# JiYuanFeng/DDP

Hardware: AMD Instinct MI355X
Metric: images/s at K DDIM steps (512x1024, 150-class) per GPU and whole node (higher is better)
Workload: dtype f32 (bf16x3-split MFMA products, fp32 accumulate); 1 GPU; ade_swin_t_k3_8x512x1024 (ADE20K Swin-T DDP decode head, 3-step DDIM, batch 8x512x1024 per GPU; x (8,256,128,256), random-init weights); images_per_call=8, ddim_steps=3, parallelism=dp1 (independent images, weights broadcast once), gemm_engine=bf16x3

## Files before the change

ddp_amd/csrc/ddp_api.hip:

```cpp
#include <stdarg.h>
#include <stdio.h>
#include <string.h>

#include <cmath>
#include <initializer_list>

#include "ddp_internal.h"

namespace ddp {

static thread_local char g_err[512] = "";

void set_error(const char* fmt, ...) {
  va_list ap;
  va_start(ap, fmt);
  vsnprintf(g_err, sizeof(g_err), fmt, ap);
  va_end(ap);
}

int check_launch(const char* what) {
  hipError_t e = hipGetLastError();
  if (e != hipSuccess) {
    set_error("%s: %s", what, hipGetErrorString(e));
    return DDP_E_LAUNCH;
// ... 515 lines not shown
  return DDP_OK;
}

int fold_affine_dev(const ddp_weights* w, int L, int S, const float* film, float* aff, hipStream_t st) {
  for (int l = 0; l < L; ++l) {
    const ddp_layer_weights& lw = w->layers[l];
    for (int s = 0; s < S; ++s) {
      float* dst = aff + (size_t(s) * L + l) * 512;
      if (lw.time_w && film) {
        DDP_TRY(launch_fold_affine(lw.norm1_w, lw.norm1_b, film + (size_t(s) * L + l) * 512, dst, 1, st));
      } else {
        DDP_TRY(launch_pack_rows(lw.norm1_w, 1, lw.norm1_b, 1, dst, 256, st));
      }
    }
  }
  return DDP_OK;
}

int prepare_geometry(const Layout& o, hipStream_t st) {
  for (int l = 0; l < o.L; ++l) DDP_TRY(launch_pos_tables(o.wcat[l], o.bcat[l], o.py[l], o.px[l], o.hh, o.wh, st));
  if (o.b3 && hipMemsetAsync(o.vpad, 0, o.vpad_floats * sizeof(float), st) != hipSuccess) {
    set_error("hipMemsetAsync(vpad) failed");
    return DDP_E_LAUNCH;
  }
  if (o.rvpad && hipMemsetAsync(o.rvpad, 0, o.vpad_floats * sizeof(float), st) != hipSuccess) {
    set_error("hipMemsetAsync(rvpad) failed");
    return DDP_E_LAUNCH;
  }
  return DDP_OK;
}

struct BiasSeg {
  int at;
  const float* src;
  int n;
};
int bias_table(float* dst, std::initializer_list<BiasSeg> segs, const char* what, hipStream_t st) {
  bool ok = hipMemsetAsync(dst, 0, size_t(b3_layer_bias_floats()) * sizeof(float), st) == hipSuccess;
  for (const BiasSeg& s : segs)
    ok = ok && (!s.src || hipMemcpyAsync(dst + s.at, s.src, size_t(s.n) * sizeof(float), hipMemcpyDeviceToDevice, st) == hipSuccess);
  if (!ok) {
    set_error("%s: bias table copy failed", what);
    return DDP_E_LAUNCH;
  }
  return DDP_OK;
}

int build_proj_images(const Layout& o, int l, unsigned char* stream, int base, hipStream_t st) {
  DDP_TRY(launch_build_stages(o.wp_v[l].p, o.wp_v[l].comp_stride, 256, 256, 1, 4, 2, base, 0, 1, 2, stream, st));
  DDP_TRY(launch_build_stages(o.wp_cat[l].p, o.wp_cat[l].comp_stride, 256, 96, 1, 1, 2, base + 8, 0, 1, 2, stream, st));
  return launch_build_stages(o.wp_cat[l].p, o.wp_cat[l].comp_stride, 256, 96, 2, 1, 1, base + 10, 64, 0, 0, stream, st);
}

int prepare_model(const ddp_cfg* c, const ddp_weights* w, const Layout& o, hipStream_t st) {
  DDP_TRY(launch_pack_cols(w->transform_w, o.Cx + o.Cm, 0, 256, o.Cx, o.wx, st));
  DDP_TRY(launch_pack_cols(w->transform_w, o.Cx + o.Cm, o.Cx, 256, o.Cm, o.wm, st));
  if (c->task == DDP_TASK_SEG) DDP_TRY(launch_build_lut(w->embedding, o.lut, o.Kc + 1, c->bit_scale, st));
  if (c->task == DDP_TASK_DEPTH) DDP_TRY(launch_pack_conv3x3(w->head_w, o.wtap, st));
  if (o.seg3) {
    if (hipMemsetAsync(o.bins_wpack, 0, size_t(256) * 2304 * sizeof(float), st) != hipSuccess ||
        hipMemsetAsync(o.bins_bias, 0, 256 * sizeof(float), st) != hipSuccess ||
        hipMemcpyAsync(o.bins_bias, w->head_b, size_t(o.Kc) * sizeof(float), hipMemcpyDeviceToDevice, st) != hipSuccess) {
      set_error("bev 3x3 conv_seg: weight copy failed");
      return DDP_E_LAUNCH;
    }
    DDP_TRY(launch_pack_conv3x3_scaled(w->head_w, nullptr, o.bins_wpack, o.Kc, 256, st));
    if (o.b3) {
      DDP_TRY(launch_split_weights(o.bins_wpack, 2304, 256, 2304, o.bins_wsplit, st));
      DDP_TRY(launch_build_stages(o.bins_wsplit, size_t(256) * 2304, 2304, 256, 0, 1, 72, 0, 2, 1, 0, o.bins_stream, st));
    }
  }
  if (o.nbins) {
    if (hipMemsetAsync(o.bins_wpack, 0, size_t(256) * 2304 * sizeof(float), st) != hipSuccess ||
        hipMemsetAsync(o.bins_bias, 0, 256 * sizeof(float), st) != hipSuccess ||
        hipMemsetAsync(o.bins_tab, 0, DDP_MAX_DEPTH_BINS * sizeof(float), st) != hipSuccess ||
        hipMemcpyAsync(o.bins_bias, w->head_b, size_t(o.nbins) * sizeof(float), hipMemcpyDeviceToDevice, st) != hipSuccess ||
        hipMemcpyAsync(o.bins_tab, w->depth_bins, size_t(o.nbins) * sizeof(float), hipMemcpyDeviceToDevice, st) != hipSuccess) {
      set_error("depth bins: weight copy failed");
      return DDP_E_LAUNCH;
    }
    DDP_TRY(launch_pack_conv3x3_scaled(w->head_w, nullptr, o.bins_wpack, o.nbins, 256, st));
    if (o.b3) {
      DDP_TRY(launch_split_weights(o.bins_wpack, 2304, 256, 2304, o.bins_wsplit, st));
      DDP_TRY(launch_build_stages(o.bins_wsplit, size_t(256) * 2304, 2304, 256, 0, 1, 72, 0, 2, 1, 0, o.bins_stream, st));
    }
  }
  for (int l = 0; l < o.L; ++l) {
    const ddp_layer_weights& lw = w->layers[l];
    DDP_TRY(launch_pack_rows(lw.sampling_offsets_w, 64, lw.attention_weights_w, 32, o.wcat[l], 256, st));
    DDP_TRY(launch_pack_rows(lw.sampling_offsets_b, 64, lw.attention_weights_b, 32, o.bcat[l], 1, st));
  }
  if (o.b3) {
    auto wr = [](const SplitW& w) { return const_cast<unsigned short*>(w.p); };
    DDP_TRY(launch_split_weights(o.wx, o.Cx, 256, o.Cx, wr(o.wp_x), st));
    if (c->task != DDP_TASK_DEPTH) DDP_TRY(launch_split_weights(o.wm, 256, 256, 256, wr(o.wp_m), st));
    if (c->task == DDP_TASK_DEPTH) DDP_TRY(launch_split_weights(o.wtap, 256, 9, 256, wr(o.wp_head), st));
    else if (!o.seg3) DDP_TRY(launch_split_weights(w->head_w, 256, o.Kc, 256, wr(o.wp_head), st));
    for (int l = 0; l < o.L; ++l) {
      const ddp_layer_weights& lw = w->layers[l];
      DDP_TRY(launch_split_weights(lw.value_proj_w, 256, 256, 256, wr(o.wp_v[l]), st));
      DDP_TRY(launch_split_weights(o.wcat[l], 256, 96, 256, wr(o.wp_cat[l]), st));
      DDP_TRY(launch_split_weights(lw.output_proj_w, 256, 256, 256, wr(o.wp_o[l]), st));
      DDP_TRY(launch_split_weights(lw.ffn0_w, 256, DDP_FFN, 256, wr(o.wp_f0[l]), st));
      DDP_TRY(launch_split_weights(lw.ffn1_w, DDP_FFN, 256, DDP_FFN, wr(o.wp_f1[l]), st));
    }
    if (c->task == DDP_TASK_SEG) {
      const int nch = (o.Kc + 63) / 64;
      DDP_TRY(launch_build_stages(o.wp_head.p, o.wp_head.comp_stride, 256, o.Kc, 1, nch, 2, 0, 0, 1, 2, o.tail_stream, st));
      DDP_TRY(bias_table(o.tail_bias, {{0, w->head_b, o.Kc}}, "seg tail", st));
      DDP_TRY(launch_build_stages(o.wp_head.p, o.wp_head.comp_stride, 256, o.Kc, 1, nch, 2, 0, 0, 1, 2, o.tail4_stream, st));
      DDP_TRY(build_proj_images(o, 0, o.tail4_stream, 2 * nch, st));
      DDP_TRY(bias_table(o.tail4_bias, {{0, w->head_b, o.Kc}, {DDP_FFN, w->layers[0].value_proj_b, 256}}, "fused tail", st));
      DDP_TRY(launch_linear(o.lut, 256, false, o.wm, 256, nullptr, nullptr, 0, 0, 0, o.tlut, 256, o.Kc + 1, 256, 256, 0, st));
    }
    if (c->task != DDP_TASK_DEPTH)
      DDP_TRY(launch_build_stages(o.wp_m.p, o.wp_m.comp_stride, 256, 256, 0, 1, 8, 0, 2, 1, 0, o.pro_stream, st));
    DDP_TRY(build_proj_images(o, 0, o.pro_stream, 8, st));
    DDP_TRY(bias_table(o.pro_bias, {{DDP_FFN, w->layers[0].value_proj_b, 256}}, "prologue", st));
    if (o.head7_stream) {
      DDP_TRY(launch_build_stages(o.wp_m.p, o.wp_m.comp_stride, 256, 256, 0, 1, 8, 0, 2, 1, 0, o.head7_stream, st));
      DDP_TRY(launch_build_stages(o.wp_x.p, o.wp_x.comp_stride, 256, 256, 0, 1, 8, 8, 2, 1, 0, o.head7_stream, st));
      if (hipMemcpyAsync(o.head7_stream + size_t(16) * 48 * 1024, o.pro_stream + size_t(8) * 48 * 1024, size_t(11) * 48 * 1024,
                         hipMemcpyDeviceToDevice, st) != hipSuccess) {
        set_error("first-step head stream copy failed");
        return DDP_E_LAUNCH;
      }
    }
    for (int l = 0; l < o.L; ++l) {
      const ddp_layer_weights& lw = w->layers[l];
      unsigned char* sp = o.wstream[l];
      DDP_TRY(launch_build_stages(o.wp_o[l].p, o.wp_o[l].comp_stride, 256, 256, 0, 1, 8, 0, 2, 1, 0, sp, st));
      DDP_TRY(launch_build_stages(o.wp_f0[l].p, o.wp_f0[l].comp_stride, 256, DDP_FFN, 1, 16, 2, 8, 0, 1, 4, sp, st));
      DDP_TRY(launch_build_stages(o.wp_f1[l].p, o.wp_f1[l].comp_stride, DDP_FFN, 256, 0, 1, 32, 10, 4, 1, 0, sp, st));
      DDP_TRY(bias_table(o.bias_ext[l], {{0, lw.ffn0_b, DDP_FFN}}, "layer", st));
      if (l + 1 < o.L) {
        DDP_TRY(build_proj_images(o, l + 1, sp, 72, st));
        if (hipMemcpyAsync(o.bias_ext[l] + DDP_FFN, w->layers[l + 1].value_proj_b, 256 * sizeof(float), hipMemcpyDeviceToDevice, st) !=
            hipSuccess) {
          set_error("bias table copy failed");
          return DDP_E_LAUNCH;
        }
      }
    }
    if (o.lt_stream && c->task != DDP_TASK_SEG && !o.seg3) {
      const size_t sb = size_t(48) * 1024;
      const int rows = c->task == DDP_TASK_DEPTH ? 9 : o.Kc;
      DDP_TRY(launch_build_stages(o.wp_head.p, o.wp_head.comp_stride, 256, rows, 1, 1, 2, 0, 0, 1, 2, o.tail_stream, st));
      DDP_TRY(bias_table(o.tail_bias, {{0, c->task == DDP_TASK_BEV ? w->head_b : nullptr, o.Kc}}, "head tail", st));
      if (hipMemcpyAsync(o.lt_stream, o.wstream[o.L - 1], 72 * sb, hipMemcpyDeviceToDevice, st) != hipSuccess ||
          hipMemcpyAsync(o.lt_stream + 72 * sb, o.tail_stream, 2 * sb, hipMemcpyDeviceToDevice, st) != hipSuccess) {
        set_error("layer + tail stream copy failed");
        return DDP_E_LAUNCH;
      }
      DDP_TRY(bias_table(o.lt_bias, {{0, w->layers[o.L - 1].ffn0_b, DDP_FFN}}, "layer + tail", st));
    }
    if (o.wvs) {
      DDP_TRY(launch_matvec(w->layers[0].value_proj_w, nullptr, o.wm, o.wvs, 256, 256, 1, 256, 256, 0, 0, st));
      DDP_TRY(launch_matvec(o.wcat[0], nullptr, o.wm, o.wvs + 256, 256, 96, 1, 256, 96, 0, 0, st));
    }
    if (o.lut64) {
      DDP_TRY(launch_build_bev_lut(w->embedding, o.lut64, o.Kc, c->bit_scale, st));
      DDP_TRY(launch_linear(o.lut64, 256, false, o.wm, 256, nullptr, nullptr, 0, 0, 0, o.tlut, 256, 1 << o.Kc, 256, 256, 0, st));
    }
    if (o.lt_stream && c->task == DDP_TASK_SEG) {
      const int nch = (o.Kc + 63) / 64;
      const size_t sb = size_t(48) * 1024;
      if (hipMemcpyAsync(o.lt_stream, o.wstream[o.L - 1], 72 * sb, hipMemcpyDeviceToDevice, st) != hipSuccess ||
          hipMemcpyAsync(o.lt_stream + 72 * sb, o.tail4_stream, size_t(2 * nch + 11) * sb, hipMemcpyDeviceToDevice, st) != hipSuccess) {
        set_error("layer + tail stream copy failed");
        return DDP_E_LAUNCH;
      }
      DDP_TRY(bias_table(o.lt_bias, {{0, w->layers[o.L - 1].ffn0_b, DDP_FFN}, {DDP_FFN, w->layers[0].value_proj_b, 256}}, "layer + tail",
                         st));
    }
  }
  return DDP_OK;
}

int publish_q(const Layout& o, const float* row_major, hipStream_t st) {
  if (o.b3 && !o.fused_layer) return launch_row_to_sb(row_major, 256, o.q_sb, int(o.M), 256, st);
  return launch_row_to_blk(row_major, o.q, int(o.M), st);
}

int conv3x3_head(const Layout& o, int n_out, int* layout, int* ld, hipStream_t st) {
  const int M = int(o.M);
  if (o.b3) {
    if (!o.fused_layer) {
      DDP_TRY(launch_sb_to_row(o.q_sb, o.s, M, 256, st));
      DDP_TRY(launch_row_to_blk(o.s, o.q, M, st));
    }
    SgemmProblem pr{};
    pr.A = o.q;
    pr.out = o.bins_logits;
    pr.stream = o.bins_stream;
    pr.M = M;
    pr.ns = 72;
    pr.conv_h = o.hh;
    pr.conv_w = o.wh;
    pr.bias = o.bins_bias;
    prof_begin(TAG_HEAD, st);
    DDP_TRY(launch_b3_sgemm(&pr, 1, 0, 1, st));
    prof_end(TAG_HEAD, st);
    *layout = 0;
    *ld = 256;
  } else {
    DDP_TRY(launch_blk_to_pad(o.q, o.bins_in, o.R, o.hh, o.wh, o.bins_guard, st));
    const int rows = o.R * (o.hh + 2) * (o.wh + 2);
    for (int t = 0; t < 9; ++t) {
      const int off = (t / 3 - 1) * (o.wh + 2) + (t % 3 - 1);
      DDP_TRY(launch_linear(o.bins_in + size_t(o.bins_guard + off) * 256, 256, false, o.bins_wpack + t * 256, 2304,
                            t == 0 ? o.bins_bias : nullptr, t == 0 ? nullptr : o.bins_logits, o.bins_ld, 0, 0, o.bins_logits,
                            o.bins_ld, rows, n_out, 256, 0, st));
    }
    *layout = 1;
    *ld = o.bins_ld;
  }
  return DDP_OK;
}

int depth_bins_head(const ddp_cfg* c, const Layout& o, float* pred, hipStream_t st) {
  DepthBinsArgs a;
// ... 1780 lines not shown
```

ddp_amd/csrc/ddp_internal.h:

```cpp
#pragma once
#include <hip/hip_runtime.h>
#include <stddef.h>
#include <atomic>
#include "../../include/ddp_mi355x.h"


#ifndef DDP_S_F32
#define DDP_S_F32 1
#endif

namespace ddp {

__device__ __forceinline__ float sigmoidf_(float x) { return 1.0f / (1.0f + expf(-x)); }

void set_error(const char* fmt, ...);
int check_launch(const char* what);

struct LdsAttrOnce {
  std::atomic<unsigned long long> done{0};
  void ensure(const void* fn, int bytes) {
    int dev = 0;
    (void)hipGetDevice(&dev);
    if (dev >= 0 && dev < 64 && ((done.load(std::memory_order_acquire) >> dev) & 1ull)) return;
    if (hipFuncSetAttribute(fn, hipFuncAttributeMaxDynamicSharedMemorySize, bytes) != hipSuccess) {
// ... 1 lines not shown
      set_error("hipFuncSetAttribute(MaxDynamicSharedMemorySize = %d) failed on device %d", bytes, dev);
      return;
    }
    if (dev >= 0 && dev < 64) done.fetch_or(1ull << dev, std::memory_order_release);
  }
};
inline int cu_count() {
  static std::atomic<int> cache[64];
  int dev = 0;
  (void)hipGetDevice(&dev);
  if (dev >= 0 && dev < 64) {
    const int c = cache[dev].load(std::memory_order_relaxed);
    if (c > 0) return c;
  }
  int n = 0;
  if (hipDeviceGetAttribute(&n, hipDeviceAttributeMultiprocessorCount, dev) != hipSuccess || n <= 0) n = 256;
  if (dev >= 0 && dev < 64) cache[dev].store(n, std::memory_order_relaxed);
  return n;
}

enum GemmTag {
  TAG_GENERIC = 0, TAG_XPROJ = 1, TAG_FEAT = 2, TAG_VALUE = 3, TAG_SAMP = 4, TAG_OUTPROJ_LN = 5, TAG_FC1 = 6,
  TAG_FC2_LN = 7, TAG_HEAD = 8, TAG_GATHER = 9, TAG_LAYER_TAIL = 10, TAG_COUNT = 11
};
void prof_begin(int tag, hipStream_t st);
void prof_end(int tag, hipStream_t st);

int launch_linear(const float* A, int lda, bool a_blk, const float* W, int ldw, const float* bias, const float* add,
                  int ld_add, int rn, int n_tok, float* out, int ldo, int M, int N, int K, int gelu, hipStream_t st,
                  int tag = TAG_GENERIC);
int launch_linear_blk(const float* A, int lda, bool a_blk, const float* W, int ldw, const float* bias,
                      const float* add, int ld_add, int rn, int n_tok, float* out_blk, int M, int N, int K, int gelu,
                      hipStream_t st);
int launch_linear_res_ln_blk(const float* A, int lda, bool a_blk, const float* W, int ldw, const float* bias,
                             const float* res_blk, const float* ga_aff, const float* be_aff, float* out_blk, int M,
                             int K, hipStream_t st);
int launch_linear_samp(const float* A_blk, const float* Wcat, const float* py, const float* px, int n_tok, int w,
                       float* out, int M, hipStream_t st);

struct SplitW {
  const unsigned short* p;
  size_t comp_stride;
};
int launch_b3_linear(const unsigned short* A_sb, const SplitW& w, const float* bias, const float* add, int ld_add,
                     int rn, int n_tok, float* out, int ldo, int M, int N, int K, hipStream_t st, int tag);
int launch_b3_linear_sb(const unsigned short* A_sb, const SplitW& w, const float* bias, const float* add, int ld_add,
                        int rn, int n_tok, unsigned short* out_sb, float* out_f32_blk, int M, int N, int K, int gelu,
                        hipStream_t st, int tag);
int launch_b3_linear_res_ln(const unsigned short* A_sb, const SplitW& w, const float* bias, const float* res_blk,
                            const unsigned short* res_sb, const float* ga_aff, const float* be_aff, float* out_f32_blk,
                            unsigned short* out_sb, int M, int K, hipStream_t st, int tag);
int launch_b3_linear_samp(const unsigned short* A_sb, const SplitW& wcat, const float* py, const float* px, int n_tok,
                          int w, float* out, int M, hipStream_t st);
int launch_build_stages(const unsigned short* Wp, size_t comp_stride, int K, int rows_valid, int tall, int n_rowblk, int n_kblk,
                        int base, int a, int b, int c, unsigned char* stream, hipStream_t st);
struct LayerLaunch {
  const unsigned short* S;
  const float* Sf;
  float* Q;
  unsigned short* Q_sb;
  const unsigned char* stream;
  const float* bias_ext;
  const float *bo, *ga0, *be0, *b2, *ga1, *be1;
  int M, has_next;
  float* v_out;
  float* samp_out;
  const float *py, *px;
  int n_tok, w;
  const float* res_f;
  const float* wm;
  const float* dvec;
};
int launch_b3_layer(const LayerLaunch& a, hipStream_t st);
struct TailLaunch {
  float* Q;
  const unsigned char* stream;
  const float* bias_ext;
  const float* lut;
  float* prob;
  unsigned short* mask_sb;
  unsigned char* x0_idx;
  const unsigned char* x0_force;
  int x0_keep;
  const float* cp_bias;
  int cp_rn;
  int M, num_classes, ldl, prob_mode;
  float alpha, sigma, alpha_next, sigma_next;
  int fuse_next;
  float* ubuf;
  const float* tlut;
  const float* res;
  int res_rn;
  int res_frag;
  float* v_out;
  float* samp_out;
  const float *py, *px;
  int n_tok, w;
  int kind;
  float threshold;
};
int launch_b3_tail(const TailLaunch& a, hipStream_t st);
bool b3_layer_tail_supported(int num_classes);
int launch_b3_layer_tail(const LayerLaunch& l, const TailLaunch& t, const unsigned char* stream, const float* bias_ext,
                         const float* seg_bias, hipStream_t st);
struct PrologueLaunch {
  const unsigned short* mask_sb;
  float* Q;
  const unsigned char* stream;
// ... 237 lines not shown
```

ddp_amd/csrc/ddp_kernels.hip:

```cpp
#include <math.h>
#include <type_traits>
#include "ddp_internal.h"

namespace ddp {

using f32x4 = __attribute__((ext_vector_type(4))) float;

namespace {

__device__ __forceinline__ float wave_sum(float v) {
#pragma unroll
  for (int o = 32; o > 0; o >>= 1) v += __shfl_xor(v, o, 64);
  return v;
}

__global__ void __launch_bounds__(256) k_nchw_to_tok(const float* __restrict__ in, float* __restrict__ out, int C,
                                                      int N) {
  __shared__ float tile[64][65];
  const int r = blockIdx.z;
  const int n0 = blockIdx.x * 64, c0 = blockIdx.y * 64;
  const int tx = threadIdx.x & 63, ty = threadIdx.x >> 6;
  const float* src = in + size_t(r) * C * N;
  float* dst = out + size_t(r) * N * C;
  for (int cc = ty; cc < 64; cc += 4) {
// ... 1 lines not shown
    tile[cc][tx] = (c < C && n < N) ? src[size_t(c) * N + n] : 0.f;
  }
  __syncthreads();
  for (int nn = ty; nn < 64; nn += 4) {
    const int n = n0 + nn, c = c0 + tx;
    if (n < N && c < C) dst[size_t(n) * C + c] = tile[tx][nn];
  }
}

__device__ __forceinline__ size_t blk_off256(int m, int ch) {
  return size_t(m >> 5) * 8192 + (ch >> 5) * 1024 + ((ch & 31) >> 3) * 256 + ((ch & 7) >> 2) * 128 + (m & 31) * 4 + (ch & 3);
}

__global__ void __launch_bounds__(256) k_row_to_blk(const float* __restrict__ in, float* __restrict__ out, int rows) {
  const int lane = threadIdx.x & 63;
  const int m = blockIdx.x * 4 + (threadIdx.x >> 6);
  if (m >= rows) return;
  const f32x4 v = *reinterpret_cast<const f32x4*>(in + size_t(m) * 256 + lane * 4);
  *reinterpret_cast<f32x4*>(out + blk_off256(m, lane * 4)) = v;
}

__device__ __forceinline__ void split3(float x, unsigned short& p1, unsigned short& p2, unsigned short& p3) {
  const unsigned xb = __float_as_uint(x);
  const unsigned hb = xb & 0xFFFF0000u;
  const float r = x - __uint_as_float(hb);
  const unsigned mb = __float_as_uint(r) & 0xFFFF0000u;
  const float r2 = r - __uint_as_float(mb);
  p1 = (unsigned short)(hb >> 16);
  p2 = (unsigned short)(mb >> 16);
  p3 = (unsigned short)(__float_as_uint(r2) >> 16);
}

__global__ void k_split_weights(const float* __restrict__ W, int ld, int rows, int K, unsigned short* __restrict__ out) {
  const int idx = blockIdx.x * blockDim.x + threadIdx.x;
  const int groups = K / 8;
  if (idx >= rows * groups) return;
  const int row = idx / groups, gq = idx - row * groups;
  const int b = gq >> 1, h = gq & 1;
  const size_t comp = size_t(rows) * K;
  unsigned short* dst = out + size_t(row) * K + 16 * b + 8 * h;
#pragma unroll
  for (int u = 0; u < 8; ++u) {
    const float x = W[size_t(row) * ld + 16 * b + 8 * (u >> 2) + 4 * h + (u & 3)];
    unsigned short p1, p2, p3;
    split3(x, p1, p2, p3);
    dst[u] = p1;
    dst[comp + u] = p2;
    dst[2 * comp + u] = p3;
  }
}

__global__ void __launch_bounds__(256) k_build_stages(const unsigned short* __restrict__ Wp, size_t comp_stride, int K,
                                                       int rows_valid, int tall, int n_kblk, int base, int a, int b, int c,
                                                       unsigned char* __restrict__ stream) {
  const int st = blockIdx.y;
  const int rowblk = st / n_kblk, kblk = st - rowblk * n_kblk;
  const int idx = blockIdx.x * 256 + threadIdx.x;
  if (idx >= 3072) return;
  const int comp = idx >> 10, rem = idx & 1023;
  int row, chunk, slot, grow, kcol;
  if (tall) {
    row = rem >> 4; chunk = rem & 15; slot = chunk ^ (row & 15);
    grow = tall == 2 ? a + (row & 31) : rowblk * 64 + row;
    kcol = (tall == 2 ? (row >> 5) : kblk) * 128 + 8 * chunk;
  } else {
    row = rem >> 2; chunk = rem & 3; slot = chunk ^ ((row >> 2) & 3);
    grow = rowblk * 256 + row;
    kcol = kblk * 32 + 8 * chunk;
  }
  uint4 v = make_uint4(0u, 0u, 0u, 0u);
  if (grow < rows_valid) v = *reinterpret_cast<const uint4*>(Wp + size_t(comp) * comp_stride + size_t(grow) * K + kcol);
  const int image = tall == 2 ? base : base + rowblk * c + (kblk >> 1) * a + (kblk & 1) * b;
  const int per_row = tall ? 16 : 4;
  *reinterpret_cast<uint4*>(stream + size_t(image) * 49152 + comp * 16384 + (row * per_row + slot) * 16) = v;
}

__global__ void __launch_bounds__(256) k_row_to_sb(const float* __restrict__ in, int ld, unsigned short* __restrict__ out,
                                                    int rows, int C) {
  const int slots = C / 8;
  const long idx = long(blockIdx.x) * blockDim.x + threadIdx.x;
  if (idx >= long(rows) * slots) return;
  const int m = int(idx / slots), sl = int(idx - long(m) * slots);
  const int b = sl >> 1, h = sl & 1;
  const float* src = in + size_t(m) * ld + 16 * b + 4 * h;
  const f32x4 lo4 = *reinterpret_cast<const f32x4*>(src);
  const f32x4 hi4 = *reinterpret_cast<const f32x4*>(src + 8);
  unsigned short p[3][8];
#pragma unroll
  for (int u = 0; u < 4; ++u) {
    split3(lo4[u], p[0][u], p[1][u], p[2][u]);
    split3(hi4[u], p[0][4 + u], p[1][4 + u], p[2][4 + u]);
  }
  char* base = reinterpret_cast<char*>(out) + size_t(m >> 5) * C * 192 + size_t(b) * 3 * 1024 + (h * 32 + (m & 31)) * 16;
#pragma unroll
  for (int c = 0; c < 3; ++c) {
    uint4 v;
    v.x = p[c][0] | (unsigned(p[c][1]) << 16);
    v.y = p[c][2] | (unsigned(p[c][3]) << 16);
    v.z = p[c][4] | (unsigned(p[c][5]) << 16);
    v.w = p[c][6] | (unsigned(p[c][7]) << 16);
    *reinterpret_cast<uint4*>(base + c * 1024) = v;
  }
}

__global__ void __launch_bounds__(256) k_nchw_to_sb(const float* __restrict__ in, unsigned short* __restrict__ out, int C, int N,
                                                     int rows) {
  __shared__ float tile[64][65];
  const int m0 = blockIdx.x * 64, c0 = blockIdx.y * 64;
  const int tx = threadIdx.x & 63, ty = threadIdx.x >> 6;
  {
    const int m = m0 + tx;
    const int r = m / N, n = m - r * N;
    const float* src = in + (size_t(r) * C + c0) * N + n;
    for (int cc = ty; cc < 64; cc += 4) tile[cc][tx] = (m < rows && c0 + cc < C) ? src[size_t(cc) * N] : 0.f;
  }
  __syncthreads();
#pragma unroll
  for (int it = 0; it < 2; ++it) {
    const int item = it * 256 + threadIdx.x;
    const int l2 = item & 63, bl = (item >> 6) & 3, gi = item >> 8;
    const int j = l2 & 31, hh = l2 >> 5;
    if (c0 + 16 * bl >= C) continue;
    unsigned short p[3][8];
#pragma unroll
    for (int u = 0; u < 8; ++u) split3(tile[16 * bl + 8 * (u >> 2) + 4 * hh + (u & 3)][gi * 32 + j], p[0][u], p[1][u], p[2][u]);
// ... 1755 lines not shown
  const int Nh = a.hh * a.wh;
  const int m = blockIdx.x * blockDim.x + threadIdx.x;
  if (m >= a.R * Nh) return;
  const float* p;
  if (a.layout == 0) {
    p = a.logits + size_t(m >> 5) * 8192 + (m & 31) * 4;
  } else {
    const int img = m / Nh, n = m - img * Nh;
    const int i = n / a.wh, j = n - i * a.wh;
    p = a.logits + (size_t(img) * (a.hh + 2) * (a.wh + 2) + size_t(i + 1) * (a.wh + 2) + (j + 1)) * a.ld;
  }
  const int K = a.num_classes, nq = (K + 3) >> 2;
  f32x4 v[8];
#pragma unroll
  for (int u = 0; u < 8; ++u) {
    const int q = u < nq ? u : nq - 1;
    const size_t off = a.layout == 0 ? size_t((q >> 1) & 3) * 256 + (q & 1) * 128 : size_t(q) * 4;
    v[u] = *reinterpret_cast<const f32x4*>(p + off);
  }
  float* pr = a.prob + size_t(m) * 32;
  float* lo = a.logits_out ? a.logits_out + size_t(m) * 32 : nullptr;
  unsigned code = 0;
#pragma unroll
  for (int u = 0; u < 8; ++u) {
    if (u >= nq) break;
    f32x4 s;
#pragma unroll
    for (int e = 0; e < 4; ++e) {
      const bool on = 4 * u + e < K;
      s[e] = on ? sigmoidf_(v[u][e]) : 0.f;
      if (u < 2 && on && s[e] > a.threshold) code |= 1u << ((4 * u + e) & 7);
    }
    if (!a.first) s += *reinterpret_cast<const f32x4*>(pr + 4 * u);
    *reinterpret_cast<f32x4*>(pr + 4 * u) = s;
    if (lo) *reinterpret_cast<f32x4*>(lo + 4 * u) = v[u];
  }
  if (a.code) a.code[m] = (unsigned char)code;
}

}

static inline int cdiv(long a, long b) { return int((a + b - 1) / b); }

int launch_nchw_to_tok(const float* in, float* out, int R, int C, int N, hipStream_t st) {
  hipLaunchKernelGGL(k_nchw_to_tok, dim3(cdiv(N, 64), cdiv(C, 64), R), dim3(256), 0, st, in, out, C, N);
  return check_launch("k_nchw_to_tok");
}
int launch_split_weights(const float* W, int ld, int rows, int K, unsigned short* out, hipStream_t st) {
  const long n = long(rows) * (K / 8);
  hipLaunchKernelGGL(k_split_weights, dim3(cdiv(n, 256)), dim3(256), 0, st, W, ld, rows, K, out);
  return check_launch("k_split_weights");
}
int launch_build_stages(const unsigned short* Wp, size_t comp_stride, int K, int rows_valid, int tall, int n_rowblk, int n_kblk,
                        int base, int a, int b, int c, unsigned char* stream, hipStream_t st) {
  hipLaunchKernelGGL(k_build_stages, dim3(12, n_rowblk * n_kblk), dim3(256), 0, st, Wp, comp_stride, K, rows_valid, tall,
                     n_kblk, base, a, b, c, stream);
  return check_launch("k_build_stages");
}
int launch_row_to_sb(const float* in, int ld, unsigned short* out_sb, int rows, int C, hipStream_t st) {
  const long n = long(rows) * (C / 8);
  hipLaunchKernelGGL(k_row_to_sb, dim3(cdiv(n, 256)), dim3(256), 0, st, in, ld, out_sb, rows, C);
  return check_launch("k_row_to_sb");
}
int launch_nchw_to_sb(const float* in, unsigned short* out_sb, int R, int C, int N, hipStream_t st) {
  const long rows = long(R) * N;
  hipLaunchKernelGGL(k_nchw_to_sb, dim3(cdiv(rows, 64), cdiv(C, 64)), dim3(256), 0, st, in, out_sb, C, N, int(rows));
  return check_launch("k_nchw_to_sb");
}
int launch_row_to_blk(const float* in, float* out_blk, int rows, hipStream_t st) {
  hipLaunchKernelGGL(k_row_to_blk, dim3(cdiv(rows, 4)), dim3(256), 0, st, in, out_blk, rows);
  return check_launch("k_row_to_blk");
}
int launch_fold_affine(const float* gamma, const float* beta, const float* film, float* out, int count, hipStream_t st) {
  if (count <= 0) return DDP_OK;
  hipLaunchKernelGGL(k_fold_affine, dim3(count), dim3(256), 0, st, gamma, beta, film, out);
  return check_launch("k_fold_affine");
}
int launch_msda_gather(const float* value, const float* samp, float* out, int rows, int n_tok, int h, int w,
                       hipStream_t st) {
  hipLaunchKernelGGL(k_msda_gather, dim3(cdiv(rows, 4)), dim3(256), 0, st, value, samp, out, rows, n_tok, h, w);
  return check_launch("k_msda_gather");
}
int launch_msda_gather_sb(const float* value, const float* samp, unsigned short* out_sb, int rows, int n_tok, int h, int w,
                          hipStream_t st) {
  hipLaunchKernelGGL(k_msda_gather_sb, dim3(cdiv(rows, 32)), dim3(64 * GSB_WAVES), 0, st, value, samp, out_sb, rows, n_tok, h, w);
  return check_launch("k_msda_gather_sb");
}
int launch_seg_postprocess(const SegPostArgs& a, hipStream_t st) {
  if (a.H == 4 * a.h && a.W == 4 * a.w && a.oh == a.ch && a.ow == a.cw && a.ch == a.H && a.cw == a.W && !a.align) {
    hipLaunchKernelGGL(k_seg_postprocess_x4, dim3(cdiv(a.w, 64), cdiv(a.h, 4), a.B), dim3(256), 0, st, a);
    return check_launch("k_seg_postprocess_x4");
  }
  hipLaunchKernelGGL(k_seg_postprocess, dim3(cdiv(a.ow, 64), cdiv(a.oh, 4), a.B), dim3(256), 0, st, a);
  return check_launch("k_seg_postprocess");
}
int launch_seg_aug_postprocess(const ddp_seg_aug* augs, int n_aug, int B, int K, int oh, int ow, int align, unsigned char* seg,
                               float* prob, hipStream_t st) {
  SegAugArgs a;
  for (int i = 0; i < n_aug; ++i) a.aug[i] = augs[i];
  a.n_aug = n_aug;
  a.B = B;
  a.K = K;
  a.oh = oh;
  a.ow = ow;
  a.align = align;
  a.seg = seg;
  a.prob = prob;
  const int lds = (2 * K * 64 + 512) * int(sizeof(float));
  static LdsAttrOnce attr;
// ... 291 lines not shown
```

ddp_amd/csrc/layer_bf16x3.h:

```cpp
#pragma once
#include <type_traits>

#include "gemm_bf16x3.h"

namespace ddp {
namespace b3 {

constexpr int LYR_BM = 128;
constexpr int LYR_THREADS = 256;
constexpr int LYR_STAGE_B = 48 * 1024;
constexpr int LYR_RING = 3;
constexpr int LYR_BIAS_OFF = LYR_RING * LYR_STAGE_B;
constexpr int LYR_BIAS_N = 1024 + 256 + 128;
constexpr int LYR_T_BO = LYR_BIAS_N, LYR_T_GA0 = LYR_T_BO + 256, LYR_T_BE0 = LYR_T_GA0 + 256, LYR_T_B2 = LYR_T_BE0 + 256,
              LYR_T_GA1 = LYR_T_B2 + 256, LYR_T_BE1 = LYR_T_GA1 + 256,
              LYR_T_SEG = LYR_T_BE1 + 256,
              LYR_TABLE_N = LYR_T_SEG + 256;
static_assert(LYR_T_SEG % 64 == 0, "bias_init addresses the table in chunks of 64 floats");
constexpr size_t LYR_LDS_B = size_t(LYR_BIAS_OFF) + LYR_TABLE_N * 4;
constexpr int LYR_ST_OUT = 8, LYR_ST_FFN = 64, LYR_ST_NEXT = 11;
constexpr int LYR_STAGES = LYR_ST_OUT + LYR_ST_FFN + LYR_ST_NEXT;

struct LayerArgs {
  const unsigned short* S;
  const float* Sf;
  float* Q;
  unsigned short* Q_sb;
  const unsigned char* stream;
  const float* bias_ext;
  const float* bo;
  const float* ga0;
  const float* be0;
  const float* b2;
  const float* ga1;
  const float* be1;
  int M;
  int has_next;
  float* v_out;
  float* samp_out;
  const float* py;
  const float* px;
  int n_tok, w;
  const float* lut;
  float* prob;
  unsigned short* mask_sb;
  unsigned char* x0_idx;
  const unsigned char* x0_force;
  int num_classes, ldl, prob_mode;
  float threshold;
  float alpha, sigma, alpha_next, sigma_next;
  const float* res;
  int res_rn;
  int res_frag;
  float* ubuf;
  const float* tlut;
  float ua, uc;
  const float* dvec;
  const float* dtaps;
  const float* dbias;
  float* dvec_rw;
  float d_min, d_max, d_bit, d_eps, d_sig, d_alpha, d_alpha_next, d_sigma_next;
  int d_scale_up;
  const float* nchw_noise;
  const float* nchw_x;
  const float* seg_bias;
  struct GemmProblem {
    const float* A;
    float* out;
    const unsigned char* stream;
    const float* bias;
    double* gn_partial;
    int M, ns, tile0, conv_h, conv_w, gn_N;
    int nchw_N;
  } gp[4];
// ... 150 lines not shown
    case 1: s.h[e1] = __uint_as_float(__float_as_uint(x(e1)) & 0xFFFF0000u); break;
    case 2: s.r[e0] = x(e0) - s.h[e0]; break;
    case 3: s.r[e1] = x(e1) - s.h[e1]; break;
    case 4: s.m[e0] = __uint_as_float(__float_as_uint(s.r[e0]) & 0xFFFF0000u); break;
    case 5: s.m[e1] = __uint_as_float(__float_as_uint(s.r[e1]) & 0xFFFF0000u); break;
    case 6: s.r[e0] = s.r[e0] - s.m[e0]; break;
    case 7: s.r[e1] = s.r[e1] - s.m[e1]; break;
    case 8: p[0][i] = __builtin_amdgcn_perm(__float_as_uint(s.h[e1]), __float_as_uint(s.h[e0]), 0x07060302); break;
    case 9: p[1][i] = __builtin_amdgcn_perm(__float_as_uint(s.m[e1]), __float_as_uint(s.m[e0]), 0x07060302); break;
    default: p[2][i] = __builtin_amdgcn_perm(__float_as_uint(s.r[e1]), __float_as_uint(s.r[e0]), 0x07060302); break;
  }
}
__device__ constexpr int SPLIT_HAND_LO[13] = {0, 3, 6, 10, 14, 17, 20, 24, 29, 33, 38, 41, 44};

#ifdef DDP_LYR_STAMP
constexpr int LYR_NSTAMP = 16;
#define DDP_LYR_STAMP_DECL unsigned long long st_prev = __builtin_readcyclecounter(), st_acc[LYR_NSTAMP] = {0, 0, 0, 0, 0, 0, 0, 0, 0, 0, 0, 0, 0, 0, 0, 0}; \
  const unsigned long long st_t0 = __builtin_amdgcn_s_memrealtime();
#define DDP_LYR_STAMP_AT(i)                                   \
  {                                                           \
    const unsigned long long st_now = __builtin_readcyclecounter(); \
    st_acc[i] += st_now - st_prev;                            \
    st_prev = st_now;                                         \
  }
#else
#define DDP_LYR_STAMP_DECL
#define DDP_LYR_STAMP_AT(i)
#endif

constexpr int LYR_NT_MIN_TOKENS = 131072;
template <bool NT>
__device__ __forceinline__ f32x4 ld_stream(const float* p) {
  if constexpr (NT) return __builtin_nontemporal_load(reinterpret_cast<const f32x4*>(p));
  else return *reinterpret_cast<const f32x4*>(p);
}
template <bool NT>
__device__ __forceinline__ void st_stream(float* p, const f32x4& v) {
  if constexpr (NT) __builtin_nontemporal_store(v, reinterpret_cast<f32x4*>(p));
  else *reinterpret_cast<f32x4*>(p) = v;
}

template <int TAG, int MODE = 0, int NCH = 0, bool NT = false, bool FORCE = false>
__global__ void __launch_bounds__(LYR_THREADS, 1)
k_layer(LayerArgs la) {
  extern __shared__ __attribute__((aligned(16))) float smem[];
  const int tid = threadIdx.x;
  int lane = tid & 63;
  const int wave = __builtin_amdgcn_readfirstlane(tid >> 6);
  int j = lane & 31;
  int h = lane >> 5;
  const int M = la.M;
  constexpr bool LT = MODE == 6 || MODE == 8 || MODE == 9;
  constexpr bool LYR = MODE == 0 || LT || MODE == 10;
  static_assert(!(MODE == 8 || MODE == 9) || NCH == 1, "the bev / depth tails are one 64-row chunk");
  const int ntiles = MODE == 5 ? la.g_tiles : (M + LYR_BM - 1) / LYR_BM;
  if (int(blockIdx.x) >= ntiles) return;
  const unsigned lds0 = (unsigned)(size_t)(lds_float_t*)smem;
  unsigned voff0 = unsigned(lane * 16), voff1 = voff0 + 4096, voff2 = voff0 + 8192;
  const unsigned wave_off = unsigned(wave * 12 * 1024);
  auto gp_of = [&](int tile) __attribute__((always_inline)) {
    return (tile >= la.gp[1].tile0 ? 1 : 0) + (tile >= la.gp[2].tile0 ? 1 : 0) + (tile >= la.gp[3].tile0 ? 1 : 0);
  };
  int fs_tile = blockIdx.x;
  int n_stages = MODE == 5 ? la.gp[gp_of(int(blockIdx.x))].ns
                       : MODE == 1 ? 2 * NCH : MODE == 4 ? 2 * NCH + LYR_ST_NEXT : MODE == 3 ? LYR_ST_NEXT : MODE == 2 ? LYR_ST_OUT + LYR_ST_NEXT
                       : LT ? LYR_ST_OUT + LYR_ST_FFN + 2 * NCH + (la.has_next ? LYR_ST_NEXT : 0)
                       : MODE == 7 ? 2 * LYR_ST_OUT + LYR_ST_NEXT
                                                                                    : (la.has_next ? LYR_STAGES : LYR_ST_OUT + LYR_ST_FFN);
  int sidx = 0;
  unsigned long long nb = 0;
  unsigned mb = 0;
  auto nxt = [](int s) { return s == LYR_RING - 1 ? 0 : s + 1; };

  const unsigned char* fs_stream = MODE == 5 ? la.gp[gp_of(int(blockIdx.x))].stream : la.stream;
  auto stage_begin = [&](int dslot) __attribute__((always_inline)) {
    const unsigned long long p = reinterpret_cast<unsigned long long>(fs_stream) + size_t(sidx) * LYR_STAGE_B + wave_off;
    const unsigned lo = __builtin_amdgcn_readfirstlane(unsigned(p)), hi = __builtin_amdgcn_readfirstlane(unsigned(p >> 32));
    nb = (static_cast<unsigned long long>(hi) << 32) | lo;
    mb = __builtin_amdgcn_readfirstlane(lds0 + unsigned(dslot * LYR_STAGE_B) + wave_off);
    if (sidx + 1 == n_stages) {
      sidx = 0;
      if constexpr (MODE == 5) {
        fs_tile += int(gridDim.x);
        const int pi = gp_of(fs_tile);
        fs_stream = la.gp[pi].stream;
        n_stages = la.gp[pi].ns;
      }
    } else {
      sidx = sidx + 1;
    }
  };
  auto dma = [&](int i0, int i1) __attribute__((always_inline)) {
#pragma unroll
    for (int i = 0; i < 12; ++i) {
      if (i < i0 || i >= i1) continue;
      switch (i) {
        case 0: stream_piece<0, 0>(nb, voff0, mb); break;
        case 1: stream_piece<1024, 0>(nb, voff0, mb); break;
        case 2: stream_piece<2048, 0>(nb, voff0, mb); break;
        case 3: stream_piece<3072, 0>(nb, voff0, mb); break;
        case 4: stream_piece<0, 4096>(nb, voff1, mb); break;
        case 5: stream_piece<1024, 4096>(nb, voff1, mb); break;
        case 6: stream_piece<2048, 4096>(nb, voff1, mb); break;
        case 7: stream_piece<3072, 4096>(nb, voff1, mb); break;
        case 8: stream_piece<0, 8192>(nb, voff2, mb); break;
        case 9: stream_piece<1024, 8192>(nb, voff2, mb); break;
// ... 728 lines not shown
        }
    }

    DDP_LYR_STAMP_AT(0)
    {
      float sum = 0.f;
#pragma unroll
      for (int t = 0; t < 8; ++t)
#pragma unroll
        for (int r = 0; r < 16; ++r) {
          const float v = acc2[t][r] + qr[t][r >> 2][r & 3];
          acc2[t][r] = v;
          sum += v;
        }
      const float mean = half_sum(sum) * (1.0f / 256.0f);
      float var = 0.f;
#pragma unroll
      for (int t = 0; t < 8; ++t)
#pragma unroll
        for (int r = 0; r < 16; ++r) {
          const float d = acc2[t][r] - mean;
          acc2[t][r] = d;
          var += d * d;
        }
      const float rstd = 1.0f / sqrtf(half_sum(var) * (1.0f / 256.0f) + 1e-5f);
#pragma unroll
      for (int t = 0; t < 8; ++t) {
#pragma unroll
        for (int g = 0; g < 4; ++g) {
          const int ch = t * 32 + 8 * g + 4 * ht;
          const f32x4 ga = *reinterpret_cast<const f32x4*>(bias_s + LYR_T_GA0 + ch);
          const f32x4 be = *reinterpret_cast<const f32x4*>(bias_s + LYR_T_BE0 + ch);
#pragma unroll
          for (int e = 0; e < 4; ++e) acc2[t][4 * g + e] = acc2[t][4 * g + e] * (rstd * ga[e]) + be[e];
        }
#pragma unroll
        for (int gp = 0; gp < 2; ++gp) {
          float xv[8];
#pragma unroll
          for (int e = 0; e < 8; ++e) xv[e] = acc2[t][8 * gp + e];
          split8_packed(xv, xa[2 * t + gp][0], xa[2 * t + gp][1], xa[2 * t + gp][2]);
        }
#pragma unroll
        for (int g = 0; g < 4; ++g) {
          const f32x4 b = *reinterpret_cast<const f32x4*>(bias_s + LYR_T_B2 + t * 32 + 8 * g + 4 * ht);
#pragma unroll
          for (int e = 0; e < 4; ++e) acc2[t][4 * g + e] += b[e];
        }
      }
    }

    DDP_LYR_STAMP_AT(1)
    refresh();
    for (int hc = 0; hc < 16; ++hc) {
      f32x16 acc1[2];
      bias_init(acc1, hc);
      tall_pair(acc1[0], acc1[1], I0);
      DDP_LYR_STAMP_AT(2)
      u32x4 hcur[3], hn[3];
      {
        float xg[8];
#pragma unroll
        for (int e = 0; e < 8; ++e) xg[e] = acc1[0][e];
        gelu_split8_packed(xg, hcur[0], hcur[1], hcur[2]);
      }
      DDP_LYR_STAMP_AT(3)
      u32x4 w[2][3];
#pragma unroll
      for (int t = 0; t < 2; ++t)
#pragma unroll
        for (int c = 0; c < 3; ++c) w[t][c] = frag2(slot, c, t, 0);
#pragma unroll
      for (int s2 = 0; s2 < 2; ++s2) {
        stage_begin(nxt(nxt(slot)));
        const int nslot = nxt(slot);
#pragma unroll
        for (int ks = 0; ks < 2; ++ks) {
          const int kb = s2 * 2 + ks;
          const int kn = kb + 1;
#pragma unroll
          for (int tpp = 0; tpp < 2; ++tpp) {
            GeluState g0, g1, g2, g3;
            const float v0 = kb < 3 ? acc1[kn >> 1][8 * (kn & 1) + 4 * tpp] : 0.f;
            const float v1 = kb < 3 ? acc1[kn >> 1][8 * (kn & 1) + 4 * tpp + 1] : 0.f;
            const float v2 = kb < 3 ? acc1[kn >> 1][8 * (kn & 1) + 4 * tpp + 2] : 0.f;
            const float v3 = kb < 3 ? acc1[kn >> 1][8 * (kn & 1) + 4 * tpp + 3] : 0.f;
            auto block = [&](auto halfc) __attribute__((always_inline)) {
              constexpr int half = decltype(halfc)::value;
              const int tp = 2 * tpp + half;
              const int blk = ks * 4 + tp;
              const bool hand = s2 == 0 && blk == 7;
              const bool nb = blk + 1 < 8 || hand;
              const int rs = hand ? nslot : slot;
              const int tp2 = hand ? 0 : (tp + 1 < 4 ? tp + 1 : 0), ks2 = hand ? 0 : (tp + 1 < 4 ? ks : ks + 1);
              if (hand) {
                __builtin_amdgcn_s_waitcnt(0x0F7B);
                __syncthreads();
              }
              auto fill = [&](auto kc) __attribute__((always_inline)) {
                constexpr int k = decltype(kc)::value;
                if (k == 0 && nb) w[0][2] = frag2(rs, 2, 2 * tp2, ks2);
                if (k == 1 && nb) w[1][2] = frag2(rs, 2, 2 * tp2 + 1, ks2);
                if (k == 4 && nb) w[0][1] = frag2(rs, 1, 2 * tp2, ks2);
                if (k == 5 && nb) w[1][1] = frag2(rs, 1, 2 * tp2 + 1, ks2);
                if (k == 10 && nb) w[0][0] = frag2(rs, 0, 2 * tp2, ks2);
                if (k == 11 && nb) w[1][0] = frag2(rs, 0, 2 * tp2 + 1, ks2);
// ... 444 lines not shown
```

Baseline: 259.6 images/s.

## Software-pipeline FFN chunks so fc1 of next chunk overlaps fc2 of current

Reorders the FFN weight-stage images so each chunk's fc1 images are streamed ahead of the previous chunk's fc2 images. The fused layer kernel (modes 0 and 10) now computes fc1 for chunk hc+1 into separate accumulators, then runs fc2 of chunk hc while interleaving the GELU of the next chunk and reading the new accumulators from AGPRs. The goal is to hide the serial fc1→GELU→fc2 dependency and the weight-DMA latency behind MFMA work. The cost is higher register and AGPR pressure and a more intricate schedule, and the last-layer streams are now rebuilt with the unreordered layout instead of being copied.

Measured after the change: 261.9 images/s, median of 6. No clear change (+0.9%).

```diff
diff --git a/ddp_amd/csrc/ddp_api.hip b/ddp_amd/csrc/ddp_api.hip
--- a/ddp_amd/csrc/ddp_api.hip
+++ b/ddp_amd/csrc/ddp_api.hip
@@ -591,6 +591,12 @@
   return launch_build_stages(o.wp_cat[l].p, o.wp_cat[l].comp_stride, 256, 96, 2, 1, 1, base + 10, 64, 0, 0, stream, st);
 }
 
+int build_layer_images(const Layout& o, int l, unsigned char* stream, int ffn_ahead, hipStream_t st) {
+  DDP_TRY(launch_build_stages(o.wp_o[l].p, o.wp_o[l].comp_stride, 256, 256, 0, 1, 8, 0, 2, 1, 0, stream, st));
+  DDP_TRY(launch_build_stages(o.wp_f0[l].p, o.wp_f0[l].comp_stride, 256, DDP_FFN, 1, 16, 2, 8, 0, 1, 4, stream, st, ffn_ahead));
+  return launch_build_stages(o.wp_f1[l].p, o.wp_f1[l].comp_stride, DDP_FFN, 256, 0, 1, 32, 10, 4, 1, 0, stream, st, ffn_ahead);
+}
+
 int prepare_model(const ddp_cfg* c, const ddp_weights* w, const Layout& o, hipStream_t st) {
   DDP_TRY(launch_pack_cols(w->transform_w, o.Cx + o.Cm, 0, 256, o.Cx, o.wx, st));
   DDP_TRY(launch_pack_cols(w->transform_w, o.Cx + o.Cm, o.Cx, 256, o.Cm, o.wm, st));
@@ -668,9 +674,7 @@
     for (int l = 0; l < o.L; ++l) {
       const ddp_layer_weights& lw = w->layers[l];
       unsigned char* sp = o.wstream[l];
-      DDP_TRY(launch_build_stages(o.wp_o[l].p, o.wp_o[l].comp_stride, 256, 256, 0, 1, 8, 0, 2, 1, 0, sp, st));
-      DDP_TRY(launch_build_stages(o.wp_f0[l].p, o.wp_f0[l].comp_stride, 256, DDP_FFN, 1, 16, 2, 8, 0, 1, 4, sp, st));
-      DDP_TRY(launch_build_stages(o.wp_f1[l].p, o.wp_f1[l].comp_stride, DDP_FFN, 256, 0, 1, 32, 10, 4, 1, 0, sp, st));
+      DDP_TRY(build_layer_images(o, l, sp, 1, st));
       DDP_TRY(bias_table(o.bias_ext[l], {{0, lw.ffn0_b, DDP_FFN}}, "layer", st));
       if (l + 1 < o.L) {
         DDP_TRY(build_proj_images(o, l + 1, sp, 72, st));
@@ -686,8 +690,8 @@
       const int rows = c->task == DDP_TASK_DEPTH ? 9 : o.Kc;
       DDP_TRY(launch_build_stages(o.wp_head.p, o.wp_head.comp_stride, 256, rows, 1, 1, 2, 0, 0, 1, 2, o.tail_stream, st));
       DDP_TRY(bias_table(o.tail_bias, {{0, c->task == DDP_TASK_BEV ? w->head_b : nullptr, o.Kc}}, "head tail", st));
-      if (hipMemcpyAsync(o.lt_stream, o.wstream[o.L - 1], 72 * sb, hipMemcpyDeviceToDevice, st) != hipSuccess ||
-          hipMemcpyAsync(o.lt_stream + 72 * sb, o.tail_stream, 2 * sb, hipMemcpyDeviceToDevice, st) != hipSuccess) {
+      DDP_TRY(build_layer_images(o, o.L - 1, o.lt_stream, 0, st));
+      if (hipMemcpyAsync(o.lt_stream + 72 * sb, o.tail_stream, 2 * sb, hipMemcpyDeviceToDevice, st) != hipSuccess) {
         set_error("layer + tail stream copy failed");
         return DDP_E_LAUNCH;
       }
@@ -704,8 +708,8 @@
     if (o.lt_stream && c->task == DDP_TASK_SEG) {
       const int nch = (o.Kc + 63) / 64;
       const size_t sb = size_t(48) * 1024;
-      if (hipMemcpyAsync(o.lt_stream, o.wstream[o.L - 1], 72 * sb, hipMemcpyDeviceToDevice, st) != hipSuccess ||
-          hipMemcpyAsync(o.lt_stream + 72 * sb, o.tail4_stream, size_t(2 * nch + 11) * sb, hipMemcpyDeviceToDevice, st) != hipSuccess) {
+      DDP_TRY(build_layer_images(o, o.L - 1, o.lt_stream, 0, st));
+      if (hipMemcpyAsync(o.lt_stream + 72 * sb, o.tail4_stream, size_t(2 * nch + 11) * sb, hipMemcpyDeviceToDevice, st) != hipSuccess) {
         set_error("layer + tail stream copy failed");
         return DDP_E_LAUNCH;
       }
diff --git a/ddp_amd/csrc/ddp_internal.h b/ddp_amd/csrc/ddp_internal.h
--- a/ddp_amd/csrc/ddp_internal.h
+++ b/ddp_amd/csrc/ddp_internal.h
@@ -77,8 +77,16 @@
                             unsigned short* out_sb, int M, int K, hipStream_t st, int tag);
 int launch_b3_linear_samp(const unsigned short* A_sb, const SplitW& wcat, const float* py, const float* px, int n_tok,
                           int w, float* out, int M, hipStream_t st);
+__host__ __device__ constexpr int ffn_ahead_image(int i) {
+  if (i < 8 || i >= 72) return i;
+  const int c = (i - 8) >> 2, fc2 = (i - 8) & 2;
+  return fc2 ? (c < 15 ? i + 2 : i) : (c > 0 ? i - 2 : i);
+}
+static_assert(ffn_ahead_image(8) == 8 && ffn_ahead_image(12) == 10 && ffn_ahead_image(10) == 12 && ffn_ahead_image(68) == 66 &&
+              ffn_ahead_image(66) == 68 && ffn_ahead_image(70) == 70 && ffn_ahead_image(71) == 71 && ffn_ahead_image(7) == 7,
+              "fc1(0) | fc1(1) fc2(0) | ... | fc1(15) fc2(14) | fc2(15)");
 int launch_build_stages(const unsigned short* Wp, size_t comp_stride, int K, int rows_valid, int tall, int n_rowblk, int n_kblk,
-                        int base, int a, int b, int c, unsigned char* stream, hipStream_t st);
+                        int base, int a, int b, int c, unsigned char* stream, hipStream_t st, int ffn_ahead = 0);
 struct LayerLaunch {
   const unsigned short* S;
   const float* Sf;
diff --git a/ddp_amd/csrc/ddp_kernels.hip b/ddp_amd/csrc/ddp_kernels.hip
--- a/ddp_amd/csrc/ddp_kernels.hip
+++ b/ddp_amd/csrc/ddp_kernels.hip
@@ -77,7 +77,7 @@
 
 __global__ void __launch_bounds__(256) k_build_stages(const unsigned short* __restrict__ Wp, size_t comp_stride, int K,
                                                        int rows_valid, int tall, int n_kblk, int base, int a, int b, int c,
-                                                       unsigned char* __restrict__ stream) {
+                                                       unsigned char* __restrict__ stream, int ffn_ahead) {
   const int st = blockIdx.y;
   const int rowblk = st / n_kblk, kblk = st - rowblk * n_kblk;
   const int idx = blockIdx.x * 256 + threadIdx.x;
@@ -95,7 +95,8 @@
   }
   uint4 v = make_uint4(0u, 0u, 0u, 0u);
   if (grow < rows_valid) v = *reinterpret_cast<const uint4*>(Wp + size_t(comp) * comp_stride + size_t(grow) * K + kcol);
-  const int image = tall == 2 ? base : base + rowblk * c + (kblk >> 1) * a + (kblk & 1) * b;
+  int image = tall == 2 ? base : base + rowblk * c + (kblk >> 1) * a + (kblk & 1) * b;
+  if (ffn_ahead) image = ffn_ahead_image(image);
   const int per_row = tall ? 16 : 4;
   *reinterpret_cast<uint4*>(stream + size_t(image) * 49152 + comp * 16384 + (row * per_row + slot) * 16) = v;
 }
@@ -1957,9 +1958,9 @@
   return check_launch("k_split_weights");
 }
 int launch_build_stages(const unsigned short* Wp, size_t comp_stride, int K, int rows_valid, int tall, int n_rowblk, int n_kblk,
-                        int base, int a, int b, int c, unsigned char* stream, hipStream_t st) {
+                        int base, int a, int b, int c, unsigned char* stream, hipStream_t st, int ffn_ahead) {
   hipLaunchKernelGGL(k_build_stages, dim3(12, n_rowblk * n_kblk), dim3(256), 0, st, Wp, comp_stride, K, rows_valid, tall,
-                     n_kblk, base, a, b, c, stream);
+                     n_kblk, base, a, b, c, stream, ffn_ahead);
   return check_launch("k_build_stages");
 }
 int launch_row_to_sb(const float* in, int ld, unsigned short* out_sb, int rows, int C, hipStream_t st) {
diff --git a/ddp_amd/csrc/layer_bf16x3.h b/ddp_amd/csrc/layer_bf16x3.h
--- a/ddp_amd/csrc/layer_bf16x3.h
+++ b/ddp_amd/csrc/layer_bf16x3.h
@@ -20,6 +20,9 @@
 constexpr size_t LYR_LDS_B = size_t(LYR_BIAS_OFF) + LYR_TABLE_N * 4;
 constexpr int LYR_ST_OUT = 8, LYR_ST_FFN = 64, LYR_ST_NEXT = 11;
 constexpr int LYR_STAGES = LYR_ST_OUT + LYR_ST_FFN + LYR_ST_NEXT;
+
+static_assert(LYR_ST_OUT == 8 && LYR_ST_FFN == 64 && ffn_ahead_image(LYR_ST_OUT + LYR_ST_FFN) == LYR_ST_OUT + LYR_ST_FFN,
+              "ffn_ahead_image: 8 output_proj images, then 16 chunks of 2 fc1 + 2 fc2 images");
 
 struct LayerArgs {
   const unsigned short* S;
@@ -276,6 +279,7 @@
   const int M = la.M;
   constexpr bool LT = MODE == 6 || MODE == 8 || MODE == 9;
   constexpr bool LYR = MODE == 0 || LT || MODE == 10;
+  constexpr bool PIPE = MODE == 0 || MODE == 10;
   static_assert(!(MODE == 8 || MODE == 9) || NCH == 1, "the bev / depth tails are one 64-row chunk");
   const int ntiles = MODE == 5 ? la.g_tiles : (M + LYR_BM - 1) / LYR_BM;
   if (int(blockIdx.x) >= ntiles) return;
@@ -1110,6 +1114,129 @@
 
     DDP_LYR_STAMP_AT(1)
     refresh();
+    if constexpr (PIPE) {
+      f32x16 acc1[2], accn[2];
+      u32x4 hcur[3];
+      auto take = [&](int i) __attribute__((always_inline)) {
+        const int f = 8 + i;
+        float v;
+        asm volatile("v_accvgpr_read_b32 %0, %1" : "=v"(v) : "a"(accn[f >> 4][f & 15]));
+        acc1[f >> 4][f & 15] = v;
+      };
+      auto wide_pair = [&]() __attribute__((always_inline)) {
+        u32x4 hn[3];
+        u32x4 w[2][3];
+#pragma unroll
+        for (int t = 0; t < 2; ++t)
+#pragma unroll
+          for (int c = 0; c < 3; ++c) w[t][c] = frag2(slot, c, t, 0);
+#pragma unroll
+        for (int s2 = 0; s2 < 2; ++s2) {
+          stage_begin(nxt(nxt(slot)));
+          const int nslot = nxt(slot);
+#pragma unroll
+          for (int ks = 0; ks < 2; ++ks) {
+            const int kb = s2 * 2 + ks;
+            const int kn = kb + 1;
+#pragma unroll
+            for (int tpp = 0; tpp < 2; ++tpp) {
+              GeluState g0, g1, g2, g3;
+              const float v0 = kb < 3 ? acc1[kn >> 1][8 * (kn & 1) + 4 * tpp] : accn[0][4 * tpp];
+              const float v1 = kb < 3 ? acc1[kn >> 1][8 * (kn & 1) + 4 * tpp + 1] : accn[0][4 * tpp + 1];
+              const float v2 = kb < 3 ? acc1[kn >> 1][8 * (kn & 1) + 4 * tpp + 2] : accn[0][4 * tpp + 2];
+              const float v3 = kb < 3 ? acc1[kn >> 1][8 * (kn & 1) + 4 * tpp + 3] : accn[0][4 * tpp + 3];
+              auto block = [&](auto halfc) __attribute__((always_inline)) {
+                constexpr int half = decltype(halfc)::value;
+                const int tp = 2 * tpp + half;
+                const int blk = ks * 4 + tp;
+                const bool hand = s2 == 0 && blk == 7;
+                const bool nb = blk + 1 < 8 || hand;
+                const int rs = hand ? nslot : slot;
+                const int tp2 = hand ? 0 : (tp + 1 < 4 ? tp + 1 : 0), ks2 = hand ? 0 : (tp + 1 < 4 ? ks : ks + 1);
+                if (hand) {
+                  __builtin_amdgcn_s_waitcnt(0x0F7B);
+                  __syncthreads();
+                }
+                auto fill = [&](auto kc) __attribute__((always_inline)) {
+                  constexpr int k = decltype(kc)::value;
+                  if (k == 0 && nb) w[0][2] = frag2(rs, 2, 2 * tp2, ks2);
+                  if (k == 1 && nb) w[1][2] = frag2(rs, 2, 2 * tp2 + 1, ks2);
+                  if (k == 4 && nb) w[0][1] = frag2(rs, 1, 2 * tp2, ks2);
+                  if (k == 5 && nb) w[1][1] = frag2(rs, 1, 2 * tp2 + 1, ks2);
+                  if (k == 10 && nb) w[0][0] = frag2(rs, 0, 2 * tp2, ks2);
+                  if (k == 11 && nb) w[1][0] = frag2(rs, 0, 2 * tp2 + 1, ks2);
+                  if (k == 3) dma(blk, blk + 1);
+                  if (k == 8 && blk < 4) dma(8 + blk, 9 + blk);
+                  {
+                    constexpr int sl = half * 12 + k;
+                    if (kb == 3) {
+                      if (sl == 4) take(12 * tpp + 0);
+                      if (sl == 5) take(12 * tpp + 1);
+                      if (sl == 7) { take(12 * tpp + 2); take(12 * tpp + 3); }
+                      if (sl == 8) { take(12 * tpp + 4); take(12 * tpp + 5); }
+                      if (sl == 20) { take(12 * tpp + 6); take(12 * tpp + 7); }
+                      if (sl == 21) { take(12 * tpp + 8); take(12 * tpp + 9); }
+                      if (sl == 22) take(12 * tpp + 10);
+                      if (sl == 23) take(12 * tpp + 11);
+                    }
+                    gelu_maybe<GELU_SCHED[sl][0]>(g0, v0);
+                    gelu_maybe<GELU_SCHED[sl][1]>(g1, v1);
+                    gelu_maybe<GELU_SCHED[sl][2]>(g2, v2);
+                    gelu_maybe<GELU_SCHED[sl][3]>(g3, v3);
+                    if (sl == 21) {
+                      hn[0][2 * tpp] = __builtin_amdgcn_perm(gelu_ph(g1), gelu_ph(g0), 0x07060302);
+                      hn[0][2 * tpp + 1] = __builtin_amdgcn_perm(gelu_ph(g3), gelu_ph(g2), 0x07060302);
+                    }
+                    if (sl == 22) {
+                      hn[1][2 * tpp] = __builtin_amdgcn_perm(gelu_pm(g1), gelu_pm(g0), 0x07060302);
+                      hn[1][2 * tpp + 1] = __builtin_amdgcn_perm(gelu_pm(g3), gelu_pm(g2), 0x07060302);
+                    }
+                    if (sl == 23) {
+                      hn[2][2 * tpp] = __builtin_amdgcn_perm(gelu_pl(g1), gelu_pl(g0), 0x07060302);
+                      hn[2][2 * tpp + 1] = __builtin_amdgcn_perm(gelu_pl(g3), gelu_pl(g2), 0x07060302);
+                    }
+                  }
+                };
+                DDP_LYR_BLOCK(acc2[2 * tp], acc2[2 * tp + 1], hcur[0], hcur[1], hcur[2], fill)
+              };
+              block(I0);
+              block(I1);
+            }
+#pragma unroll
+            for (int c = 0; c < 3; ++c) hcur[c] = hn[c];
+          }
+          if (s2 == 1) {
+            wait_vm12();
+            __syncthreads();
+          }
+          slot = nxt(slot);
+        }
+      };
+      bias_init(accn, 0);
+      asm volatile("" : "+a"(accn[0]), "+a"(accn[1]));
+      tall_pair(accn[0], accn[1], I0);
+      DDP_LYR_STAMP_AT(2)
+      {
+        float xg[8];
+#pragma unroll
+        for (int e = 0; e < 8; ++e) xg[e] = accn[0][e];
+        gelu_split8_packed(xg, hcur[0], hcur[1], hcur[2]);
+#pragma unroll
+        for (int i = 0; i < 24; ++i) take(i);
+      }
+      DDP_LYR_STAMP_AT(3)
+#pragma unroll 1
+      for (int hc = 0; hc < 15; ++hc) {
+        bias_init(accn, hc + 1);
+        asm volatile("" : "+a"(accn[0]), "+a"(accn[1]));
+        tall_pair(accn[0], accn[1], I0);
+        DDP_LYR_STAMP_AT(2)
+        wide_pair();
+        DDP_LYR_STAMP_AT(4)
+      }
+      wide_pair();
+      DDP_LYR_STAMP_AT(4)
+    } else
     for (int hc = 0; hc < 16; ++hc) {
       f32x16 acc1[2];
       bias_init(acc1, hc);
```
